# Jisu-Linnea-Han/ClimateMachine.jl

Hardware: AMD Instinct MI355X
Metric: DG RHS DOF-updates/sec (higher is better)
Workload: dtype f64; 1 GPU; Held-Suarez dry GCM (BASELINE configs[2]), stacked cubed sphere 6x30x30x8 elements, N=4, LSRK54 explicit, hyperdiffusion (DryBiharmonic, horizontal), Rusanov, fp64; elements=43200, nodes_per_element=125, states=5, parallelism=element partition (Hilbert, whole columns), 1 rank(s), RCCL p2p halo

## Files before the change

climatemachine.jl_amd/csrc/cmdg.hip:

```cpp
#include <dlfcn.h>

#include <algorithm>
#include <new>
#include <tuple>

#include "lapfused_tables.h"
#include "rccl.h"
#include "stepping.h"

namespace cmdg {

namespace {
typedef int (*roctx_push_t)(const char *);
typedef int (*roctx_pop_t)();
roctx_push_t g_roctx_push = nullptr;
roctx_pop_t g_roctx_pop = nullptr;
int g_roctx_state = 0;
void roctx_resolve()
{
    g_roctx_state = -1;
    const char *names[] = {"librocprofiler-sdk-roctx.so.1", "librocprofiler-sdk-roctx.so", "libroctx64.so.4",
                           "libroctx64.so", nullptr};
    const char *want = getenv("CMDG_ROCTX");
    void *lib = nullptr;
// ... 95 lines not shown
        m.first->eng->err.clear();
    }
    dev.emplace(named[0].first->eng);
}

int GroupCall::finish(int rc)
{
    if (rc == CMDG_OK) return rc;
    std::string msg = cmdg_status_string(rc);
    for (auto &m : members)
        if (!m.first->eng->err.empty()) {
            msg = m.second + m.first->eng->err;
            break;
        }
    for (auto &m : members) m.first->err = msg;
    return rc;
}

EngineBase::~EngineBase()
{
    delete worker;
    worker = nullptr;
    if (s_comp) hipStreamSynchronize(s_comp);
    if (s_comm) hipStreamSynchronize(s_comm);
    prof_collect();
    if (graph_exec) hipGraphExecDestroy(graph_exec);
    if (nccl_comm && rccl::CommDestroy) rccl::CommDestroy(nccl_comm);
}

static __global__ void k_face_digest(const double *__restrict__ vgeo, int nvgeo,
                                     const double *__restrict__ sgeo,
                                     const int64_t *__restrict__ vmapM,
                                     const int64_t *__restrict__ vmapP,
                                     const int64_t *__restrict__ elemtobndy, int NQ, int NQV,
                                     int64_t nreal, int32_t *__restrict__ faceP,
                                     double *__restrict__ faceG, double *__restrict__ faceW,
                                     int32_t *__restrict__ facePr, int *__restrict__ bad)
{
    const int Np = NQ * NQ * NQV, Nfph = NQ * NQV, Nfpv = NQ * NQ;
    const int Nfp = Nfph > Nfpv ? Nfph : Nfpv, NFT = 4 * Nfph + 2 * Nfpv;
    const int64_t I = (int64_t)blockIdx.x * blockDim.x + threadIdx.x;
    if (I >= nreal * NFT) return;
    const int64_t e = I / NFT;
    const int t = (int)(I % NFT);
    int f, n;
    if (t < 4 * Nfph) {
        f = t / Nfph;
        n = t % Nfph;
    } else {
        f = 4 + (t - 4 * Nfph) / Nfpv;
        n = (t - 4 * Nfph) % Nfpv;
    }
    const int64_t o = n + (int64_t)Nfp * (f + 6 * e);
    const int a = n % NQ, b = n / NQ;
    int vid;
    switch (f) {
    case 0: vid = NQ * (a + NQ * b); break;
    case 1: vid = (NQ - 1) + NQ * (a + NQ * b); break;
    case 2: vid = a + NQ * NQ * b; break;
    case 3: vid = a + NQ * ((NQ - 1) + NQ * b); break;
    case 4: vid = n; break;
    default: vid = n + NQ * NQ * (NQV - 1); break;
    }
    int flags = 0;
    const int64_t idM = vmapM[o] - 1;
    if (idM != e * Np + vid) flags |= 1;
    int64_t idP = vmapP[o] - 1;
    if (elemtobndy[f + 6 * e] != 0) idP = e * Np + vid;
    if (idP < 0 || idP > 2147483647LL) flags |= 4;
    faceP[I] = (int32_t)idP;
    const int64_t eP = idP >= 0 ? idP / Np : 0;
    facePr[I] = (int32_t)(eP * Np + ring_slot_of(NQ, NQV, (int)(idP - eP * Np)));
    const double *sg = sgeo + 5 * o;
#pragma unroll
    for (int c = 0; c < 4; ++c) faceG[((int64_t)4 * e + c) * NFT + t] = sg[c];
    const double mi = vgeo[vid + (int64_t)Np * (VMI + (int64_t)nvgeo * e)];
    if (!(sg[SVMI] == mi)) flags |= 2;
    faceW[I] = mi * sg[SSM];
    if (flags) atomicOr(bad, flags);
}

static __global__ void k_lapfused_fill(const double *__restrict__ vgeo, int nvgeo, const int32_t *__restrict__ faceP,
                                       const double *__restrict__ faceG, const double *__restrict__ faceW,
                                       const int32_t *__restrict__ lapI, int Np, int NFT, int NL, int64_t nreal,
                                       double *__restrict__ lapT)
{
    const int64_t I = (int64_t)blockIdx.x * blockDim.x + threadIdx.x;
    if (I >= nreal * NL) return;
    const int64_t e = I / NL;
    const int t = (int)(I % NL);
    const int64_t idP = faceP[NFT * e + t], N = idP / Np;
    const int vidP = (int)(idP - N * Np), tP = lapI[(2 * e + 0) * NL + t];
    const double *vg = vgeo + (int64_t)Np * nvgeo * N + vidP;
    const int rows[6] = {XI1X1, XI1X2, XI1X3, XI2X1, XI2X2, XI2X3};
    double *dst = lapT + 10 * e * NL + t;
#pragma unroll
    for (int c = 0; c < 6; ++c) dst[(int64_t)c * NL] = vg[(int64_t)rows[c] * Np];
#pragma unroll
    for (int c = 0; c < 3; ++c) dst[(int64_t)(6 + c) * NL] = faceG[((int64_t)4 * N + c) * NFT + tP];
    dst[(int64_t)9 * NL] = faceW[NFT * N + tP];
}

int EngineBase::init_lapfused()
{
    if (!garg_capable() || ngl <= 0 || nhyp != 3 * ngl || diffusion_direction != DIR_HORIZONTAL || nghost != 0 ||
        communicate() || fv || esdg || nreal < 1)
        return CMDG_OK;
    const int NFT = 4 * NQ * NQV + 2 * NQ * NQ, NL = 4 * NQ * NQV;
    std::vector<int32_t> h_faceP((size_t)(nreal * NFT));
    std::vector<int64_t> h_bndy((size_t)(6 * nreal));
    HIPCHK(hipMemcpy(h_faceP.data(), d_faceP, sizeof(int32_t) * h_faceP.size(), hipMemcpyDeviceToHost));
    HIPCHK(hipMemcpy(h_bndy.data(), g.elemtobndy, sizeof(int64_t) * h_bndy.size(), hipMemcpyDeviceToHost));
    LapFusedTables tab;
    lapfused_build(NQ, NQV, nreal, h_faceP.data(), h_bndy.data(), tab);
    if (!tab.eligible) return CMDG_OK;
    std::vector<int32_t> h_lapI((size_t)(2 * NL * nreal));
    for (int64_t e = 0; e < nreal; ++e)
        for (int t = 0; t < NL; ++t) {
            h_lapI[(size_t)((2 * e + 0) * NL + t)] = tab.tP[(size_t)(NL * e + t)];
            h_lapI[(size_t)((2 * e + 1) * NL + t)] = tab.tE[(size_t)(NL * e + t)];
        }
    HIPCHK(d_lapI.alloc(h_lapI.size()));
    HIPCHK(d_lapT.alloc((size_t)(10 * NL * nreal)));
    HIPCHK(hipMemcpy(d_lapI, h_lapI.data(), sizeof(int32_t) * h_lapI.size(), hipMemcpyHostToDevice));
    hipLaunchKernelGGL(k_lapfused_fill, dim3((unsigned)((nreal * NL + 255) / 256)), dim3(256), 0, s_comp, g.vgeo,
                       g.nvgeo, d_faceP.get(), d_faceG.get(), d_faceW.get(), d_lapI.get(), Np, NFT, NL, nreal,
                       d_lapT.get());
    if (hipGetLastError() != hipSuccess || hipStreamSynchronize(s_comp) != hipSuccess)
        return fail(CMDG_ERR_HIP, "cmdg_create: the tables of the fused Laplacian pass failed");
    lapfused_ok = true;
    return CMDG_OK;
}

int EngineBase::init(const cmdg_desc *d)
{
    Np = NQ * NQ * NQV;
    Nfp = NQ * (NQ > NQV ? NQ : NQV);
    if (d->N[0] != d->N[1] || d->N[0] != NQ - 1 || d->N[2] != NQV - 1)
        return fail(CMDG_ERR_INVALID, "cmdg_create: polynomial orders do not match the engine");
    if (NQV != NQ && !d->Dv)
        return fail(CMDG_ERR_INVALID, "cmdg_create: Dv is required when the vertical order differs");
    nreal = d->nreal;
    nghost = d->nghost;
    nelem = nreal + nghost;
    nf_first = d->nf_first;
    direction = d->direction;
    diffusion_direction = d->diffusion_direction;
    stacked = d->stacked;
    if (!d->vgeo || !d->sgeo || !d->vmapM || !d->vmapP || !d->elemtobndy || !d->D ||
        !d->state_auxiliary)
        return fail(CMDG_ERR_INVALID, "cmdg_create: a required grid/state pointer is NULL");
    if (d->nvgeo < 11) return fail(CMDG_ERR_INVALID, "cmdg_create: vgeo needs >= 11 columns");
    if (d->ninterior + d->nexterior != nreal)
        return fail(CMDG_ERR_INVALID, "cmdg_create: interior + exterior != nreal");
    if ((d->ninterior > 0 && !d->interiorelems) || (d->nexterior > 0 && !d->exteriorelems))
        return fail(CMDG_ERR_INVALID, "cmdg_create: element list pointer is NULL");
    if (direction < 0 || direction > 2 || diffusion_direction < 0 || diffusion_direction > 2)
        return fail(CMDG_ERR_INVALID, "cmdg_create: bad direction");
    g.vgeo = d->vgeo;
    g.sgeo = d->sgeo;
    g.vmapM = d->vmapM;
    g.vmapP = d->vmapP;
    g.elemtobndy = d->elemtobndy;
    g.nvgeo = d->nvgeo;
    d_interior = d_interior_user = d->interiorelems;
    ninterior = d->ninterior;
    d_exterior = d_exterior_user = d->exteriorelems;
    nexterior = d->nexterior;
    d_activedofs = d->activedofs;
    d_vmapsend = d->vmapsend;
    nvmapsend = d->nvmapsend;
    d_vmaprecv = d->vmaprecv;
    nvmaprecv = d->nvmaprecv;
    if (d->nnabr > 0) {
        if (!d->nabrtorank || !d->nabrtovmapsend || !d->nabrtovmaprecv || !d->vmapsend ||
            !d->vmaprecv)
            return fail(CMDG_ERR_INVALID, "cmdg_create: halo tables missing");
        nabrtorank.assign(d->nabrtorank, d->nabrtorank + d->nnabr);
        nabrsend.assign(d->nabrtovmapsend, d->nabrtovmapsend + 2 * d->nnabr);
        nabrrecv.assign(d->nabrtovmaprecv, d->nabrtovmaprecv + 2 * d->nnabr);
    }
    HIPCHK(hipGetDevice(&dev));
    HIPCHK(s_comp.create(hipStreamNonBlocking));
    {
        int lo = 0, hi = 0;
        const char *pv = getenv("CMDG_HALO_PRIORITY");
        if (communicate() && pv && *pv == '1' && hipDeviceGetStreamPriorityRange(&lo, &hi) == hipSuccess && hi < lo)
            HIPCHK(s_comm.create(hipStreamNonBlocking, hi));
        else
            HIPCHK(s_comm.create(hipStreamNonBlocking));
    }
    for (int i = 0; i < 2; ++i) {
        HIPCHK(ev_int[i].create(hipEventDisableTiming));
        HIPCHK(ev_ext[i].create(hipEventDisableTiming));
    }
    HIPCHK(gev_fork.create(hipEventDisableTiming));
    if (const char *v = getenv("CMDG_STEP_GRAPH")) step_graph = *v && *v != '0';
    HIPCHK(ev_comp.create(hipEventDisableTiming));
    HIPCHK(d_D.alloc(NQ * NQ));
    HIPCHK(hipMemcpy(d_D, d->D, sizeof(double) * NQ * NQ, hipMemcpyHostToDevice));
    g.D = d_D;
    g.Dv = d_D;
    if (NQV != NQ) {
        HIPCHK(d_Dv.alloc(NQV * NQV));
        HIPCHK(hipMemcpy(d_Dv, d->Dv, sizeof(double) * NQV * NQV, hipMemcpyHostToDevice));
        g.Dv = d_Dv;
    }
    {
        const int NFT = 4 * NQ * NQV + 2 * NQ * NQ;
// ... 764 lines not shown
```

climatemachine.jl_amd/csrc/kernels.h:

```cpp
#pragma once
#include "cmdg_common.h"
#include "law_defaults.h"

#ifndef CMDG_TEND_MINW
#define CMDG_TEND_MINW 1
#endif
#ifndef CMDG_TEND_EPB_LARGE
#define CMDG_TEND_EPB_LARGE 2
#endif
#ifndef CMDG_TEND_EPB_SMALL
#define CMDG_TEND_EPB_SMALL 1
#endif
#ifndef CMDG_GRAD_MINW
#define CMDG_GRAD_MINW 4
#endif
#ifndef CMDG_GRAD_BOUND_LARGE
#define CMDG_GRAD_BOUND_LARGE 1024
#endif
#ifndef CMDG_LAP_MINW
#define CMDG_LAP_MINW 1
#endif
#ifndef CMDG_LAPFUSED_MINW
#define CMDG_LAPFUSED_MINW 4
#endif
#ifndef CMDG_LAPFUSED_STAGE
#define CMDG_LAPFUSED_STAGE(idx, dep) asm volatile("" : "+v"(idx) : "v"(dep))
#endif

namespace cmdg {

template <class P>
struct PassArgs {
    typename P::Params prm;
    GridDev g;
    const int64_t *elems;
    int64_t nelems;
    const double *Q;
    const double *aux;
    double *aux_rw;
    const double *derived;
    double *gf;
    double *hypgrad;
    double *hypdiv;
    double *tendency;
    double *Qout;
    double *garg;
    double *lapr;
    int hypdiv_out;
    double t, alpha, beta;
    const double *tptr;
    double rkb_dt, rka_next;
    int direction;
    int model_dir;
    int nf_first;
    HaloDev h;
};

struct FacePt {
    double n[3], sM, vMI;
    double w;
    int64_t eP;
    int vidM, vidP, bctag;
};

template <int NQ, int NQV = NQ>
__host__ __device__ __forceinline__ constexpr int face_vid(int f, int n)
{
    const int a = n % NQ, b = n / NQ;
    switch (f) {
    case 0: return NQ * (a + NQ * b);
    case 1: return (NQ - 1) + NQ * (a + NQ * b);
    case 2: return a + NQ * NQ * b;
    case 3: return a + NQ * ((NQ - 1) + NQ * b);
    case 4: return n;
    default: return n + NQ * NQ * (NQV - 1);
    }
}

template <int NQ, int NQV = NQ>
__device__ __forceinline__ void face_index(const GridDev &g, int64_t e, int t, int f, int32_t &idP,
                                           int &bctag)
{
    idP = g.faceP[(int64_t)KDims<NQ, NQV>::NFT * e + t];
    bctag = (int)g.elemtobndy[f + 6 * e];
}
template <int NQ, int NQV = NQ, bool LIFTW = false>
__device__ __forceinline__ void face_geometry(const GridDev &g, int64_t e, int t, int f, int n,
                                              int32_t idP, int bctag, FacePt &fp)
{
    constexpr int Np = KDims<NQ, NQV>::Np, NFT = KDims<NQ, NQV>::NFT;
    const double *sg = g.faceG + (int64_t)4 * NFT * e + t;
    fp.n[0] = sg[0];
    fp.n[1] = sg[NFT];
    fp.n[2] = sg[2 * NFT];
    fp.vidM = face_vid<NQ, NQV>(f, n);
    if constexpr (LIFTW) {
        fp.w = g.faceW[(int64_t)NFT * e + t];
    } else {
        fp.sM = sg[3 * NFT];
        fp.vMI = g.vgeo[fp.vidM + (int64_t)Np * (VMI + (int64_t)g.nvgeo * e)];
    }
    fp.bctag = bctag;
    fp.eP = idP / Np;
    fp.vidP = idP - (int)fp.eP * Np;
}
template <int NQ, int NQV = NQ, bool LIFTW = false>
__device__ __forceinline__ void face_setup(const GridDev &g, int64_t e, int t, int f, int n,
                                           FacePt &fp)
{
// ... 793 lines not shown
                sC[(1 * NG + s) * Np + tid] = contravariant(M, x21, x22, x23, G1, G2, G3);
            }
            if (vt) sC[(2 * NG + s) * Np + tid] = contravariant(M, x31, x32, x33, G1, G2, G3);
            const int sidx = surf_index<NQ, NQV>(tid);
            if (sidx >= 0) {
                sM[(3 * s + 0) * NSURF + sidx] = G1;
                sM[(3 * s + 1) * NSURF + sidx] = G2;
                sM[(3 * s + 2) * NSURF + sidx] = G3;
            }
        }
    }
    __syncthreads();
    if (tid < Np) {
        const int i = tid % NQ, j = (tid / NQ) % NQ, k = tid / (NQ * NQ);
#pragma unroll
        for (int s = 0; s < NGL; ++s) {
            double dh = 0.0, dv = 0.0;
            if (hz) dh = div_volume_h<NQ>(MI, sD, sC + (0 * NG + s) * Np, sC + (1 * NG + s) * Np, i, j, k);
            if (vt) {
#pragma unroll
                for (int kk = 0; kk < NQV; ++kk)
                    dv -= MI * sDv[kk + NQV * k] * sC[(2 * NG + s) * Np + i + NQ * (j + NQ * kk)];
            }
            sA[s * Np + tid] = hz ? (vt ? dh + dv : dh) : dv;
        }
    }
    __syncthreads();
    Vec<NGL> corr;
    int vidM = 0, fpair = -1;
    if (tid < KD::NFT) {
        int f, n;
        KD::face_task(tid, f, n);
        const bool on = f < 4 ? hz : vt;
        if (on) {
            FacePt fp;
            face_setup<NQ, NQV, true>(a.g, e, tid, f, n, fp);
            Vec<NHG> gM, gP;
            const int sidx = surf_index<NQ, NQV>(fp.vidM);
#pragma unroll
            for (int q = 0; q < NHG; ++q) gM[q] = sM[q * NSURF + sidx];
            load_plus_hg<NHG, Np, NHG>(gP, a.hypgrad, a.h.recvHG, ghost_slot<Np>(a.h, fp.eP, fp.vidP),
                                    fp.vidP, fp.eP);
            if (fp.bctag != 0) {
                Vec<NAUX> auxM, auxP;
                load_state<NAUX, Np>(auxM, a.aux, fp.vidM, e);
                load_state<NAUX, Np>(auxP, a.aux, fp.vidP, fp.eP);
                P::boundary_state_divergence(a.prm, fp.bctag, gP, auxP, fp.n, gM, auxM, a_t);
            }
            const double nh0 = fp.n[0] / 2, nh1 = fp.n[1] / 2, nh2 = fp.n[2] / 2;
#pragma unroll
            for (int s = 0; s < NGL; ++s) {
                const double ldiv = central_divergence_flux(&gP[3 * s], &gM[3 * s], nh0, nh1, nh2);
                corr[s] = fp.w * ldiv;
            }
            vidM = fp.vidM;
            fpair = f / 2;
        }
    }
#pragma unroll
    for (int p = 0; p < 3; ++p) {
        if (fpair == p) {
#pragma unroll
            for (int s = 0; s < NGL; ++s) sA[s * Np + vidM] += corr[s];
        }
        __syncthreads();
    }
    if constexpr (RING) store_ring_major<NG, NQ, NQV>(a.lapr, e, tid, (int)blockDim.x, sA);
    if (tid < Np) {
        if (!RING || a.hypdiv_out) {
#pragma unroll
            for (int s = 0; s < NGL; ++s)
                a.hypdiv[tid + (int64_t)Np * (s + (int64_t)NHYP * e)] = sA[s * Np + tid];
        }
    }
    if constexpr (NGL > 0)
        send_nodes<NGL, NGL>(a.h, 0, e, tid, (int)blockDim.x, [&](int s, int n) { return sA[s * Np + n]; });
}

template <class P, int NQ, int NQV = NQ>
__global__ void __launch_bounds__((KDims<NQ, NQV>::NT), CMDG_LAPFUSED_MINW) k_lapfused(const PassArgs<P> a)
{
    using KD = KDims<NQ, NQV>;
    constexpr int Np = KD::Np, NGL = P::NGL, NHG = 3 * NGL, NHYP = P::NHYP, NG = NGL > 0 ? NGL : 1,
                  NFT = KD::NFT, NL = 4 * KD::Nfph, NT = KD::NT;
    static_assert(NT >= NL && NGL > 0, "one lane per lateral face task");
    __shared__ double sD[NQ * NQ];
    __shared__ double sG[NG * Np];
    __shared__ double sA[3 * NG * Np];
    __shared__ double sC[2 * NG * Np];
    __shared__ double sL[NG * Np];
    const int tid = threadIdx.x;
    const int64_t e = a.elems[xcd_remap(blockIdx.x, gridDim.x)] - 1;
    const int ft = tid - (NT - NL);
    if (tid < NQ * NQ) sD[tid] = a.g.D[tid];
    if (tid < Np) {
        const double *rec = a.garg + garg_at<NGL, Np>(tid, e);
        Vec<NGL> r;
#pragma unroll
        for (int s = 0; s < NGL; ++s) r[s] = rec[s];
#pragma unroll
        for (int s = 0; s < NGL; ++s) sG[s * Np + tid] = r[s];
    }
    FacePt fp;
    int tP = 0, tE = -1, iP = 0, jP = 0, kP = 0;
    int32_t idE = 0;
    const double *gN = a.garg;
    if (ft >= 0) {
        int f, n;
        KD::face_task(ft, f, n);
        face_setup<NQ, NQV, true>(a.g, e, ft, f, n, fp);
        tP = a.g.facePr[((int64_t)2 * e + 0) * NL + ft];
        tE = a.g.facePr[((int64_t)2 * e + 1) * NL + ft];
        gN = a.garg + garg_at<NGL, Np>(0, fp.eP);
        iP = fp.vidP % NQ, jP = (fp.vidP / NQ) % NQ, kP = fp.vidP / (NQ * NQ);
        if (tE >= 0) idE = a.g.faceP[(int64_t)NFT * fp.eP + tE];
    }
    double M = 0, MI = 0, x11 = 0, x12 = 0, x13 = 0, x21 = 0, x22 = 0, x23 = 0;
    if (tid < Np) {
        const double *vg = a.g.vgeo + (int64_t)Np * a.g.nvgeo * e + tid;
        M = vg[VM * Np];
        MI = vg[VMI * Np];
        x11 = vg[XI1X1 * Np], x12 = vg[XI1X2 * Np], x13 = vg[XI1X3 * Np];
        x21 = vg[XI2X1 * Np], x22 = vg[XI2X2 * Np], x23 = vg[XI2X3 * Np];
    }
    __syncthreads();
    if (tid < Np) {
        const int i = tid % NQ, j = (tid / NQ) % NQ, k = tid / (NQ * NQ);
        Vec<NHG> gh;
        gh.negzero();
#pragma unroll
        for (int s = 0; s < NGL; ++s)
            grad_volume_h<NQ>(
                sD, i, j, [&](int n) { return sG[s * Np + n + NQ * (j + NQ * k)]; },
                [&](int n) { return sG[s * Np + i + NQ * (n + NQ * k)]; }, x11, x12, x13, x21, x22, x23, &gh[3 * s]);
#pragma unroll
        for (int q = 0; q < NHG; ++q) sA[q * Np + tid] = gh[q];
    }
    Vec<NHG> corr, gP;
    int fpair = -1;
    if (ft >= 0) {
        fpair = ft / (2 * KD::Nfph);
        const double *lapT = a.derived + (int64_t)10 * NL * e + ft;
        Vec<NGL> GY, G1, G2;
        double r1[NQ][NG];
#pragma unroll
        for (int s = 0; s < NGL; ++s) GY[s] = gN[NGL * fp.vidP + s];
#pragma unroll
        for (int n = 0; n < NQ; ++n)
#pragma unroll
            for (int s = 0; s < NGL; ++s) r1[n][s] = gN[NGL * (n + NQ * (jP + NQ * kP)) + s];
#pragma unroll
        for (int s = 0; s < NGL; ++s) G1[s] = line_derivative<NQ>(sD, iP, [&](int n) { return r1[n][s]; });
#pragma unroll
        for (int s = 0; s < NGL; ++s) CMDG_LAPFUSED_STAGE(kP, G1[s]);
        double r2[NQ][NG];
#pragma unroll
        for (int n = 0; n < NQ; ++n)
#pragma unroll
            for (int s = 0; s < NGL; ++s) r2[n][s] = gN[NGL * (iP + NQ * (n + NQ * kP)) + s];
        double T[6];
#pragma unroll
        for (int c = 0; c < 6; ++c) T[c] = lapT[c * NL];
#pragma unroll
        for (int s = 0; s < NGL; ++s) G2[s] = line_derivative<NQ>(sD, jP, [&](int n) { return r2[n][s]; });
        gP.negzero();
#pragma unroll
        for (int s = 0; s < NGL; ++s) metric_gradient(T[0], T[1], T[2], T[3], T[4], T[5], G1[s], G2[s], &gP[3 * s]);
#pragma unroll
        for (int q = 0; q < NHG; ++q) CMDG_LAPFUSED_STAGE(idE, gP[q]);
        double nS[3], wS, nE[3] = {0, 0, 0}, wE = 0;
#pragma unroll
        for (int d = 0; d < 3; ++d) nS[d] = lapT[(6 + d) * NL];
        wS = lapT[9 * NL];
        Vec<NGL> GE;
        int pairE = 2;
        if (tE >= 0) {
            const double *sg = a.g.faceG + (int64_t)4 * NFT * fp.eP + tE;
            nE[0] = sg[0], nE[1] = sg[NFT], nE[2] = sg[2 * NFT];
            wE = a.g.faceW[(int64_t)NFT * fp.eP + tE];
            const double *rec = a.garg + (int64_t)NGL * idE;
#pragma unroll
            for (int s = 0; s < NGL; ++s) GE[s] = rec[s];
            int fE, nn;
            KD::face_task(tE, fE, nn);
            pairE = fE / 2;
        }
        int fS, nn;
        KD::face_task(tP, fS, nn);
        const bool edge_first = pairE < fS / 2;
        Vec<NGL> GM;
#pragma unroll
        for (int s = 0; s < NGL; ++s) GM[s] = sG[s * Np + fp.vidM];
#pragma unroll
        for (int s = 0; s < NGL; ++s)
#pragma unroll
            for (int d = 0; d < 3; ++d) {
                const double lS = gradient_lift(wS, central_gradient_flux(nS[d], GM[s], GY[s]), nS[d] * GY[s]);
                if (tE >= 0) {
                    const double lE = gradient_lift(wE, central_gradient_flux(nE[d], GE[s], GY[s]), nE[d] * GY[s]);
                    gP[3 * s + d] += edge_first ? lE : lS;
                    gP[3 * s + d] += edge_first ? lS : lE;
                } else {
                    gP[3 * s + d] += lS;
                }
            }
#pragma unroll
        for (int s = 0; s < NGL; ++s)
#pragma unroll
            for (int d = 0; d < 3; ++d)
                corr[3 * s + d] =
                    gradient_lift(fp.w, central_gradient_flux(fp.n[d], GY[s], GM[s]), fp.n[d] * GM[s]);
    }
    __syncthreads();
#pragma unroll
    for (int p = 0; p < 2; ++p) {
        if (fpair == p) {
#pragma unroll
            for (int q = 0; q < NHG; ++q) sA[q * Np + fp.vidM] += corr[q];
        }
        __syncthreads();
    }
    if (tid < Np) {
#pragma unroll
        for (int s = 0; s < NGL; ++s) {
            const double G1 = sA[(3 * s + 0) * Np + tid], G2 = sA[(3 * s + 1) * Np + tid],
                         G3 = sA[(3 * s + 2) * Np + tid];
            sC[(0 * NG + s) * Np + tid] = contravariant(M, x11, x12, x13, G1, G2, G3);
            sC[(1 * NG + s) * Np + tid] = contravariant(M, x21, x22, x23, G1, G2, G3);
        }
    }
    __syncthreads();
    if (tid < Np) {
        const int i = tid % NQ, j = (tid / NQ) % NQ, k = tid / (NQ * NQ);
#pragma unroll
        for (int s = 0; s < NGL; ++s)
            sL[s * Np + tid] = div_volume_h<NQ>(MI, sD, sC + (0 * NG + s) * Np, sC + (1 * NG + s) * Np, i, j, k);
    }
    Vec<NGL> corrL;
    if (ft >= 0) {
        Vec<NHG> gM;
#pragma unroll
        for (int q = 0; q < NHG; ++q) gM[q] = sA[q * Np + fp.vidM];
        const double nh0 = fp.n[0] / 2, nh1 = fp.n[1] / 2, nh2 = fp.n[2] / 2;
#pragma unroll
        for (int s = 0; s < NGL; ++s) {
            const double ldiv = central_divergence_flux(&gP[3 * s], &gM[3 * s], nh0, nh1, nh2);
            corrL[s] = fp.w * ldiv;
        }
    }
    __syncthreads();
#pragma unroll
    for (int p = 0; p < 2; ++p) {
        if (fpair == p) {
#pragma unroll
            for (int s = 0; s < NGL; ++s) sL[s * Np + fp.vidM] += corrL[s];
        }
        __syncthreads();
    }
    store_ring_major<NG, NQ, NQV>(a.lapr, e, tid, (int)blockDim.x, sL);
    if (tid < Np && a.hypdiv_out) {
#pragma unroll
        for (int s = 0; s < NGL; ++s) a.hypdiv[tid + (int64_t)Np * (s + (int64_t)NHYP * e)] = sL[s * Np + tid];
    }
}

template <class P, int NQ, int NQV = NQ, bool RING = false>
__global__ void __launch_bounds__((KDims<NQ, NQV>::NT), CMDG_LAP_MINW) k_gradlap(const PassArgs<P> a)
{
    using KD = KDims<NQ, NQV>;
    const double a_t = a.tptr ? *a.tptr : a.t;
    constexpr int Np = KD::Np, NS = P::NS, NAUX = P::NAUX, NGL = P::NGL,
                  NHG = 3 * NGL, NHYP = P::NHYP, NG = NGL > 0 ? NGL : 1,
                  NH = NHYP > 0 ? NHYP : 1;
    __shared__ double sD[NQ * NQ + (NQV == NQ ? 0 : NQV * NQV)];
    const double *const sDv = sD + (NQV == NQ ? 0 : NQ * NQ);
    __shared__ double sL[NG * Np];
    __shared__ double sA[NH * Np];
    const int tid = threadIdx.x;
    const int64_t e = a.elems[xcd_remap(blockIdx.x, gridDim.x)] - 1;
    if (tid < NQ * NQ) sD[tid] = a.g.D[tid];
    if constexpr (NQV != NQ) {
        if (tid < NQV * NQV) sD[NQ * NQ + tid] = a.g.Dv[tid];
    }
    const bool hz = a.direction != DIR_VERTICAL, vt = a.direction != DIR_HORIZONTAL;
    if (tid < Np) {
        Vec<NGL> l;
        if constexpr (RING) {
            const double *rec = a.lapr + garg_at<NG, Np>(ring_slot<NQ, NQV>(tid), e);
#pragma unroll
            for (int s = 0; s < NGL; ++s) l[s] = rec[s];
        } else {
#pragma unroll
            for (int s = 0; s < NGL; ++s) l[s] = a.hypdiv[tid + (int64_t)Np * (s + (int64_t)NHYP * e)];
        }
#pragma unroll
        for (int s = 0; s < NGL; ++s) sL[s * Np + tid] = l[s];
    }
    __syncthreads();
    if (tid < Np) {
        const int i = tid % NQ, j = (tid / NQ) % NQ, k = tid / (NQ * NQ);
        const double *vg = a.g.vgeo + (int64_t)Np * a.g.nvgeo * e + tid;
        Vec<NS> lQ;
        Vec<NAUX> laux;
        load_state<NS, Np>(lQ, a.Q, tid, e);
        load_state<NAUX, Np>(laux, a.aux, tid, e);
        Vec<NHG> lh, lv;
        lh.negzero();
        lv.negzero();
        if (hz) {
            const double x11 = vg[XI1X1 * Np], x12 = vg[XI1X2 * Np], x13 = vg[XI1X3 * Np];
            const double x21 = vg[XI2X1 * Np], x22 = vg[XI2X2 * Np], x23 = vg[XI2X3 * Np];
#pragma unroll
            for (int s = 0; s < NGL; ++s) {
                double l1 = 0.0, l2 = 0.0;
#pragma unroll
                for (int n = 0; n < NQ; ++n) {
                    l1 += sD[i + NQ * n] * sL[s * Np + n + NQ * (j + NQ * k)];
                    l2 += sD[j + NQ * n] * sL[s * Np + i + NQ * (n + NQ * k)];
                }
                lh[3 * s + 0] = x11 * l1;
                lh[3 * s + 1] = x12 * l1;
                lh[3 * s + 2] = x13 * l1;
// ... 322 lines not shown
```

climatemachine.jl_amd/csrc/lapfused_tables.h:

```cpp
#pragma once
#include <stdint.h>

#include <string>
#include <vector>

namespace cmdg {

struct LapFusedTables {
    int NQ = 0, NQV = 0;
    int64_t nreal = 0;
    bool eligible = false;
    std::string why;
    std::vector<int32_t> tP, tE;
};

inline int lapfused_face_vid(int NQ, int NQV, int t)
{
    const int Nfph = NQ * NQV, f = t / Nfph, n = t % Nfph, a = n % NQ, b = n / NQ;
    switch (f) {
    case 0: return NQ * (a + NQ * b);
    case 1: return (NQ - 1) + NQ * (a + NQ * b);
    case 2: return a + NQ * NQ * b;
    default: return a + NQ * ((NQ - 1) + NQ * b);
    }
}

inline void lapfused_tasks_of(int NQ, int NQV, int vid, int out[2])
{
    const int Nfph = NQ * NQV, i = vid % NQ, j = (vid / NQ) % NQ, k = vid / (NQ * NQ);
    out[0] = i == 0 ? j + NQ * k : (i == NQ - 1 ? Nfph + j + NQ * k : -1);
    out[1] = j == 0 ? 2 * Nfph + i + NQ * k : (j == NQ - 1 ? 3 * Nfph + i + NQ * k : -1);
}

inline void lapfused_build(int NQ, int NQV, int64_t nreal, const int32_t *faceP, const int64_t *elemtobndy,
                           LapFusedTables &out)
{
    out = LapFusedTables();
    out.NQ = NQ;
    out.NQV = NQV;
    out.nreal = nreal;
    auto no = [&](const std::string &m) {
        out.eligible = false;
        out.why = m;
        out.tP.clear();
        out.tE.clear();
    };
    if (NQ < 2 || NQV < 1 || nreal < 1 || !faceP || !elemtobndy) return no("empty grid");
    const int Np = NQ * NQ * NQV, Nfph = NQ * NQV, NL = 4 * Nfph, NFT = NL + 2 * NQ * NQ;
    auto str = [](int64_t v) { return std::to_string(v); };
    for (int64_t e = 0; e < nreal; ++e)
        for (int f = 0; f < 4; ++f)
            if (elemtobndy[f + 6 * e] != 0)
                return no("lateral face " + str(f + 1) + " of element " + str(e + 1) + " is a boundary face");
    out.tP.assign((size_t)(NL * nreal), -1);
    out.tE.assign((size_t)(NL * nreal), -1);
    for (int64_t e = 0; e < nreal; ++e)
        for (int t = 0; t < NL; ++t) {
            const int64_t idP = faceP[NFT * e + t];
            const int64_t me = e * Np + lapfused_face_vid(NQ, NQV, t);
            if (idP < 0 || idP >= nreal * Np)
                return no("face task " + str(t) + " of element " + str(e + 1) + " has no real element on its plus side");
            const int64_t N = idP / Np;
            int cand[2];
            lapfused_tasks_of(NQ, NQV, (int)(idP - N * Np), cand);
            int found = -1, other = -1, matches = 0;
            for (int c = 0; c < 2; ++c) {
                if (cand[c] < 0) continue;
                if (faceP[NFT * N + cand[c]] == me) {
                    if (matches++ == 0) found = cand[c];
                } else {
                    other = cand[c];
                }
            }
            if (matches != 1)
                return no("face task " + str(t) + " of element " + str(e + 1) + (matches == 0 ? " is not seen" : " is seen twice") +
                          " from its neighbour " + str(N + 1));
            out.tP[(size_t)(NL * e + t)] = found;
            out.tE[(size_t)(NL * e + t)] = other;
        }
    out.eligible = true;
}

}
```

Measured before the change: 22.05 billion DOF-updates/s.

## Share neighbour face-row values via LDS and precompute edge geometry in fused Laplacian

The fused Laplacian kernel now loads only the neighbour's normal line per face lane and shares the along-face values through a new LDS buffer, so the tangential derivative comes from LDS instead of a second strided global gather. Edge-neighbour normals, weights and record indices are precomputed into the per-element table, replacing the dependent faceP/faceG lookups at run time. Loads are hoisted ahead of the first barrier, and the manual asm staging macros are replaced with simple register pins. The host builder adds checks that each face row maps to a single neighbour row, which could make some grids ineligible for this path, and the extra LDS buffer may change occupancy.

Result: faster. 22.54 billion DOF-updates/s (median of 6 runs) (+2.2%).

```diff
diff --git a/climatemachine.jl_amd/csrc/cmdg.hip b/climatemachine.jl_amd/csrc/cmdg.hip
--- a/climatemachine.jl_amd/csrc/cmdg.hip
+++ b/climatemachine.jl_amd/csrc/cmdg.hip
@@ -201,23 +201,30 @@
 
 static __global__ void k_lapfused_fill(const double *__restrict__ vgeo, int nvgeo, const int32_t *__restrict__ faceP,
                                        const double *__restrict__ faceG, const double *__restrict__ faceW,
-                                       const int32_t *__restrict__ lapI, int Np, int NFT, int NL, int64_t nreal,
-                                       double *__restrict__ lapT)
-{
+                                       const int32_t *__restrict__ lapI, const int32_t *__restrict__ tE_of, int NQ,
+                                       int NQV, int64_t nreal, double *__restrict__ lapT)
+{
+    const int Np = NQ * NQ * NQV, Nfph = NQ * NQV, NL = 4 * Nfph, NFT = NL + 2 * NQ * NQ, NE = 8 * NQV;
     const int64_t I = (int64_t)blockIdx.x * blockDim.x + threadIdx.x;
     if (I >= nreal * NL) return;
     const int64_t e = I / NL;
     const int t = (int)(I % NL);
     const int64_t idP = faceP[NFT * e + t], N = idP / Np;
-    const int vidP = (int)(idP - N * Np), tP = lapI[(2 * e + 0) * NL + t];
+    const int vidP = (int)(idP - N * Np), tP = lapI[(2 * e + 0) * NL + t], tE = tE_of[I];
     const double *vg = vgeo + (int64_t)Np * nvgeo * N + vidP;
     const int rows[6] = {XI1X1, XI1X2, XI1X3, XI2X1, XI2X2, XI2X3};
-    double *dst = lapT + 10 * e * NL + t;
+    double *dst = lapT + (int64_t)(10 * NL + 4 * NE) * e + t;
 #pragma unroll
     for (int c = 0; c < 6; ++c) dst[(int64_t)c * NL] = vg[(int64_t)rows[c] * Np];
 #pragma unroll
     for (int c = 0; c < 3; ++c) dst[(int64_t)(6 + c) * NL] = faceG[((int64_t)4 * N + c) * NFT + tP];
     dst[(int64_t)9 * NL] = faceW[NFT * N + tP];
+    if (tE < 0) return;
+    const bool last = lapfused_index_in_face(NQ, tP / Nfph, vidP) == NQ - 1;
+    double *edge = lapT + (int64_t)(10 * NL + 4 * NE) * e + 10 * NL + lapfused_edge_slot(NQV, t / Nfph, (t % Nfph) / NQ, last);
+#pragma unroll
+    for (int c = 0; c < 3; ++c) edge[c * NE] = faceG[((int64_t)4 * N + c) * NFT + tE];
+    edge[3 * NE] = faceW[NFT * N + tE];
 }
 
 int EngineBase::init_lapfused()
@@ -237,13 +244,16 @@
     for (int64_t e = 0; e < nreal; ++e)
         for (int t = 0; t < NL; ++t) {
             h_lapI[(size_t)((2 * e + 0) * NL + t)] = tab.tP[(size_t)(NL * e + t)];
-            h_lapI[(size_t)((2 * e + 1) * NL + t)] = tab.tE[(size_t)(NL * e + t)];
-        }
+            h_lapI[(size_t)((2 * e + 1) * NL + t)] = tab.idE[(size_t)(NL * e + t)];
+        }
+    DevBuf<int32_t> d_tE;
     HIPCHK(d_lapI.alloc(h_lapI.size()));
-    HIPCHK(d_lapT.alloc((size_t)(10 * NL * nreal)));
+    HIPCHK(d_tE.alloc(tab.tE.size()));
+    HIPCHK(d_lapT.alloc((size_t)((10 * NL + 4 * 8 * NQV) * nreal)));
     HIPCHK(hipMemcpy(d_lapI, h_lapI.data(), sizeof(int32_t) * h_lapI.size(), hipMemcpyHostToDevice));
+    HIPCHK(hipMemcpy(d_tE, tab.tE.data(), sizeof(int32_t) * tab.tE.size(), hipMemcpyHostToDevice));
     hipLaunchKernelGGL(k_lapfused_fill, dim3((unsigned)((nreal * NL + 255) / 256)), dim3(256), 0, s_comp, g.vgeo,
-                       g.nvgeo, d_faceP.get(), d_faceG.get(), d_faceW.get(), d_lapI.get(), Np, NFT, NL, nreal,
+                       g.nvgeo, d_faceP.get(), d_faceG.get(), d_faceW.get(), d_lapI.get(), d_tE.get(), NQ, NQV, nreal,
                        d_lapT.get());
     if (hipGetLastError() != hipSuccess || hipStreamSynchronize(s_comp) != hipSuccess)
         return fail(CMDG_ERR_HIP, "cmdg_create: the tables of the fused Laplacian pass failed");
diff --git a/climatemachine.jl_amd/csrc/kernels.h b/climatemachine.jl_amd/csrc/kernels.h
--- a/climatemachine.jl_amd/csrc/kernels.h
+++ b/climatemachine.jl_amd/csrc/kernels.h
@@ -22,9 +22,6 @@
 #endif
 #ifndef CMDG_LAPFUSED_MINW
 #define CMDG_LAPFUSED_MINW 4
-#endif
-#ifndef CMDG_LAPFUSED_STAGE
-#define CMDG_LAPFUSED_STAGE(idx, dep) asm volatile("" : "+v"(idx) : "v"(dep))
 #endif
 
 namespace cmdg {
@@ -984,46 +981,66 @@
 {
     using KD = KDims<NQ, NQV>;
     constexpr int Np = KD::Np, NGL = P::NGL, NHG = 3 * NGL, NHYP = P::NHYP, NG = NGL > 0 ? NGL : 1,
-                  NFT = KD::NFT, NL = 4 * KD::Nfph, NT = KD::NT;
+                  NL = 4 * KD::Nfph, NT = KD::NT, NE = 8 * NQV, LT = 10 * NL + 4 * NE;
     static_assert(NT >= NL && NGL > 0, "one lane per lateral face task");
     __shared__ double sD[NQ * NQ];
     __shared__ double sG[NG * Np];
     __shared__ double sA[3 * NG * Np];
     __shared__ double sC[2 * NG * Np];
     __shared__ double sL[NG * Np];
+    __shared__ double sX[NG * NL];
+    static_assert(sizeof(double) * (NQ * NQ + 7 * NG * Np + NG * NL) <= 32768,
+                  "LDS of k_lapfused: five work-groups per CU");
     const int tid = threadIdx.x;
     const int64_t e = a.elems[xcd_remap(blockIdx.x, gridDim.x)] - 1;
     const int ft = tid - (NT - NL);
     if (tid < NQ * NQ) sD[tid] = a.g.D[tid];
+    Vec<NGL> r;
+    double M = 0, MI = 0, x11 = 0, x12 = 0, x13 = 0, x21 = 0, x22 = 0, x23 = 0;
+#pragma unroll
+    for (int s = 0; s < NGL; ++s) r[s] = 0;
     if (tid < Np) {
         const double *rec = a.garg + garg_at<NGL, Np>(tid, e);
-        Vec<NGL> r;
 #pragma unroll
         for (int s = 0; s < NGL; ++s) r[s] = rec[s];
-#pragma unroll
-        for (int s = 0; s < NGL; ++s) sG[s * Np + tid] = r[s];
-    }
-    FacePt fp;
-    int tP = 0, tE = -1, iP = 0, jP = 0, kP = 0;
-    int32_t idE = 0;
-    const double *gN = a.garg;
+        const double *vg = a.g.vgeo + (int64_t)Np * a.g.nvgeo * e + tid;
+        M = vg[VM * Np];
+        MI = vg[VMI * Np];
+        x11 = vg[XI1X1 * Np], x12 = vg[XI1X2 * Np], x13 = vg[XI1X3 * Np];
+        x21 = vg[XI2X1 * Np], x22 = vg[XI2X2 * Np], x23 = vg[XI2X3 * Np];
+    }
+    FacePt fp = {};
+    int32_t idE = -1;
+    int tP = 0;
     if (ft >= 0) {
         int f, n;
         KD::face_task(ft, f, n);
         face_setup<NQ, NQV, true>(a.g, e, ft, f, n, fp);
         tP = a.g.facePr[((int64_t)2 * e + 0) * NL + ft];
-        tE = a.g.facePr[((int64_t)2 * e + 1) * NL + ft];
-        gN = a.garg + garg_at<NGL, Np>(0, fp.eP);
-        iP = fp.vidP % NQ, jP = (fp.vidP / NQ) % NQ, kP = fp.vidP / (NQ * NQ);
-        if (tE >= 0) idE = a.g.faceP[(int64_t)NFT * fp.eP + tE];
-    }
-    double M = 0, MI = 0, x11 = 0, x12 = 0, x13 = 0, x21 = 0, x22 = 0, x23 = 0;
+        idE = a.g.facePr[((int64_t)2 * e + 1) * NL + ft];
+    }
+    asm volatile("" ::"v"(M), "v"(MI), "v"(x11), "v"(x12), "v"(x13), "v"(x21), "v"(x22), "v"(x23), "v"(r[0]),
+                 "v"(r[NGL - 1]), "v"(fp.vidP), "v"(fp.w), "v"(fp.n[0]), "v"(fp.n[1]), "v"(fp.n[2]), "v"(tP), "v"(idE));
     if (tid < Np) {
-        const double *vg = a.g.vgeo + (int64_t)Np * a.g.nvgeo * e + tid;
-        M = vg[VM * Np];
-        MI = vg[VMI * Np];
-        x11 = vg[XI1X1 * Np], x12 = vg[XI1X2 * Np], x13 = vg[XI1X3 * Np];
-        x21 = vg[XI2X1 * Np], x22 = vg[XI2X2 * Np], x23 = vg[XI2X3 * Np];
+#pragma unroll
+        for (int s = 0; s < NGL; ++s) sG[s * Np + tid] = r[s];
+    }
+    int idx = 0, xrow = 0;
+    bool x1 = true, far = false;
+    double rn[NQ][NG] = {};
+    if (ft >= 0) {
+        int fS, nn;
+        KD::face_task(tP, fS, nn);
+        x1 = fS < 2, far = fS & 1;
+        const int iP = fp.vidP % NQ, jP = (fp.vidP / NQ) % NQ, kP = fp.vidP / (NQ * NQ);
+        idx = x1 ? jP : iP;
+        xrow = ft - ft % NQ;
+        const double *line = a.garg + garg_at<NGL, Np>(x1 ? NQ * (jP + NQ * kP) : iP + NQ * NQ * kP, fp.eP);
+        const int step = x1 ? NGL : NGL * NQ;
+#pragma unroll
+        for (int m = 0; m < NQ; ++m)
+#pragma unroll
+            for (int s = 0; s < NGL; ++s) rn[m][s] = line[m * step + s];
     }
     __syncthreads();
     if (tid < Np) {
@@ -1038,67 +1055,92 @@
 #pragma unroll
         for (int q = 0; q < NHG; ++q) sA[q * Np + tid] = gh[q];
     }
-    Vec<NHG> corr, gP;
+    Vec<NHG> corr;
+    Vec<NGL> Gn;
     int fpair = -1;
     if (ft >= 0) {
         fpair = ft / (2 * KD::Nfph);
-        const double *lapT = a.derived + (int64_t)10 * NL * e + ft;
-        Vec<NGL> GY, G1, G2;
-        double r1[NQ][NG];
-#pragma unroll
-        for (int s = 0; s < NGL; ++s) GY[s] = gN[NGL * fp.vidP + s];
-#pragma unroll
-        for (int n = 0; n < NQ; ++n)
-#pragma unroll
-            for (int s = 0; s < NGL; ++s) r1[n][s] = gN[NGL * (n + NQ * (jP + NQ * kP)) + s];
-#pragma unroll
-        for (int s = 0; s < NGL; ++s) G1[s] = line_derivative<NQ>(sD, iP, [&](int n) { return r1[n][s]; });
-#pragma unroll
-        for (int s = 0; s < NGL; ++s) CMDG_LAPFUSED_STAGE(kP, G1[s]);
-        double r2[NQ][NG];
-#pragma unroll
-        for (int n = 0; n < NQ; ++n)
-#pragma unroll
-            for (int s = 0; s < NGL; ++s) r2[n][s] = gN[NGL * (iP + NQ * (n + NQ * kP)) + s];
-        double T[6];
-#pragma unroll
-        for (int c = 0; c < 6; ++c) T[c] = lapT[c * NL];
-#pragma unroll
-        for (int s = 0; s < NGL; ++s) G2[s] = line_derivative<NQ>(sD, jP, [&](int n) { return r2[n][s]; });
+        Vec<NGL> GY, GM;
+#pragma unroll
+        for (int s = 0; s < NGL; ++s) GY[s] = far ? rn[NQ - 1][s] : rn[0][s];
+#pragma unroll
+        for (int s = 0; s < NGL; ++s) sX[s * NL + xrow + idx] = GY[s];
+#pragma unroll
+        for (int s = 0; s < NGL; ++s) GM[s] = sG[s * Np + fp.vidM];
+#pragma unroll
+        for (int s = 0; s < NGL; ++s)
+            Gn[s] = line_derivative<NQ>(sD, far ? NQ - 1 : 0, [&](int m) { return rn[m][s]; });
+#pragma unroll
+        for (int s = 0; s < NGL; ++s)
+#pragma unroll
+            for (int d = 0; d < 3; ++d)
+                corr[3 * s + d] =
+                    gradient_lift(fp.w, central_gradient_flux(fp.n[d], GY[s], GM[s]), fp.n[d] * GM[s]);
+    }
+    __syncthreads();
+#pragma unroll
+    for (int m = 0; m < NQ; ++m) asm volatile("" ::"v"(rn[m][0]), "v"(rn[m][NGL - 1]));
+#pragma unroll
+    for (int p = 0; p < 2; ++p) {
+        if (fpair == p) {
+#pragma unroll
+            for (int q = 0; q < NHG; ++q) sA[q * Np + fp.vidM] += corr[q];
+        }
+        __syncthreads();
+    }
+    double T[10], nE[3] = {0, 0, 0}, wE = 0;
+    Vec<NGL> GE;
+    if (ft >= 0) {
+        const double *lapT = a.derived + (int64_t)LT * e;
+#pragma unroll
+        for (int c = 0; c < 10; ++c) T[c] = lapT[c * NL + ft];
+        if (idE >= 0) {
+            const double *edge = lapT + 10 * NL + 2 * (ft / NQ) + (idx == NQ - 1 ? 1 : 0);
+            nE[0] = edge[0], nE[1] = edge[NE], nE[2] = edge[2 * NE];
+            wE = edge[3 * NE];
+            const double *rec = a.garg + (int64_t)NGL * idE;
+#pragma unroll
+            for (int s = 0; s < NGL; ++s) GE[s] = rec[s];
+        }
+    }
+    if (tid < Np) {
+#pragma unroll
+        for (int s = 0; s < NGL; ++s) {
+            const double G1 = sA[(3 * s + 0) * Np + tid], G2 = sA[(3 * s + 1) * Np + tid],
+                         G3 = sA[(3 * s + 2) * Np + tid];
+            sC[(0 * NG + s) * Np + tid] = contravariant(M, x11, x12, x13, G1, G2, G3);
+            sC[(1 * NG + s) * Np + tid] = contravariant(M, x21, x22, x23, G1, G2, G3);
+        }
+    }
+    __syncthreads();
+    if (tid < Np) {
+        const int i = tid % NQ, j = (tid / NQ) % NQ, k = tid / (NQ * NQ);
+#pragma unroll
+        for (int s = 0; s < NGL; ++s)
+            sL[s * Np + tid] = div_volume_h<NQ>(MI, sD, sC + (0 * NG + s) * Np, sC + (1 * NG + s) * Np, i, j, k);
+    }
+    Vec<NGL> corrL;
+    if (ft >= 0) {
+        Vec<NGL> GY, GM, Gf;
+#pragma unroll
+        for (int s = 0; s < NGL; ++s) GY[s] = sX[s * NL + xrow + idx];
+#pragma unroll
+        for (int s = 0; s < NGL; ++s) GM[s] = sG[s * Np + fp.vidM];
+#pragma unroll
+        for (int s = 0; s < NGL; ++s)
+            Gf[s] = line_derivative<NQ>(sD, idx, [&](int m) { return sX[s * NL + xrow + m]; });
+        Vec<NHG> gP;
         gP.negzero();
 #pragma unroll
-        for (int s = 0; s < NGL; ++s) metric_gradient(T[0], T[1], T[2], T[3], T[4], T[5], G1[s], G2[s], &gP[3 * s]);
-#pragma unroll
-        for (int q = 0; q < NHG; ++q) CMDG_LAPFUSED_STAGE(idE, gP[q]);
-        double nS[3], wS, nE[3] = {0, 0, 0}, wE = 0;
-#pragma unroll
-        for (int d = 0; d < 3; ++d) nS[d] = lapT[(6 + d) * NL];
-        wS = lapT[9 * NL];
-        Vec<NGL> GE;
-        int pairE = 2;
-        if (tE >= 0) {
-            const double *sg = a.g.faceG + (int64_t)4 * NFT * fp.eP + tE;
-            nE[0] = sg[0], nE[1] = sg[NFT], nE[2] = sg[2 * NFT];
-            wE = a.g.faceW[(int64_t)NFT * fp.eP + tE];
-            const double *rec = a.garg + (int64_t)NGL * idE;
-#pragma unroll
-            for (int s = 0; s < NGL; ++s) GE[s] = rec[s];
-            int fE, nn;
-            KD::face_task(tE, fE, nn);
-            pairE = fE / 2;
-        }
-        int fS, nn;
-        KD::face_task(tP, fS, nn);
-        const bool edge_first = pairE < fS / 2;
-        Vec<NGL> GM;
-#pragma unroll
-        for (int s = 0; s < NGL; ++s) GM[s] = sG[s * Np + fp.vidM];
-#pragma unroll
         for (int s = 0; s < NGL; ++s)
+            metric_gradient(T[0], T[1], T[2], T[3], T[4], T[5], x1 ? Gn[s] : Gf[s], x1 ? Gf[s] : Gn[s], &gP[3 * s]);
+        const bool edge_first = !x1;
+#pragma unroll
+        for (int s = 0; s < NGL; ++s)
 #pragma unroll
             for (int d = 0; d < 3; ++d) {
-                const double lS = gradient_lift(wS, central_gradient_flux(nS[d], GM[s], GY[s]), nS[d] * GY[s]);
-                if (tE >= 0) {
+                const double lS = gradient_lift(T[9], central_gradient_flux(T[6 + d], GM[s], GY[s]), T[6 + d] * GY[s]);
+                if (idE >= 0) {
                     const double lE = gradient_lift(wE, central_gradient_flux(nE[d], GE[s], GY[s]), nE[d] * GY[s]);
                     gP[3 * s + d] += edge_first ? lE : lS;
                     gP[3 * s + d] += edge_first ? lS : lE;
@@ -1106,40 +1148,6 @@
                     gP[3 * s + d] += lS;
                 }
             }
-#pragma unroll
-        for (int s = 0; s < NGL; ++s)
-#pragma unroll
-            for (int d = 0; d < 3; ++d)
-                corr[3 * s + d] =
-                    gradient_lift(fp.w, central_gradient_flux(fp.n[d], GY[s], GM[s]), fp.n[d] * GM[s]);
-    }
-    __syncthreads();
-#pragma unroll
-    for (int p = 0; p < 2; ++p) {
-        if (fpair == p) {
-#pragma unroll
-            for (int q = 0; q < NHG; ++q) sA[q * Np + fp.vidM] += corr[q];
-        }
-        __syncthreads();
-    }
-    if (tid < Np) {
-#pragma unroll
-        for (int s = 0; s < NGL; ++s) {
-            const double G1 = sA[(3 * s + 0) * Np + tid], G2 = sA[(3 * s + 1) * Np + tid],
-                         G3 = sA[(3 * s + 2) * Np + tid];
-            sC[(0 * NG + s) * Np + tid] = contravariant(M, x11, x12, x13, G1, G2, G3);
-            sC[(1 * NG + s) * Np + tid] = contravariant(M, x21, x22, x23, G1, G2, G3);
-        }
-    }
-    __syncthreads();
-    if (tid < Np) {
-        const int i = tid % NQ, j = (tid / NQ) % NQ, k = tid / (NQ * NQ);
-#pragma unroll
-        for (int s = 0; s < NGL; ++s)
-            sL[s * Np + tid] = div_volume_h<NQ>(MI, sD, sC + (0 * NG + s) * Np, sC + (1 * NG + s) * Np, i, j, k);
-    }
-    Vec<NGL> corrL;
-    if (ft >= 0) {
         Vec<NHG> gM;
 #pragma unroll
         for (int q = 0; q < NHG; ++q) gM[q] = sA[q * Np + fp.vidM];
diff --git a/climatemachine.jl_amd/csrc/lapfused_tables.h b/climatemachine.jl_amd/csrc/lapfused_tables.h
--- a/climatemachine.jl_amd/csrc/lapfused_tables.h
+++ b/climatemachine.jl_amd/csrc/lapfused_tables.h
@@ -3,6 +3,12 @@
 
 #include <string>
 #include <vector>
+
+#ifdef __HIPCC__
+#define CMDG_LAPFUSED_HD __host__ __device__
+#else
+#define CMDG_LAPFUSED_HD
+#endif
 
 namespace cmdg {
 
@@ -12,7 +18,17 @@
     bool eligible = false;
     std::string why;
     std::vector<int32_t> tP, tE;
+    std::vector<int32_t> idE;
 };
+
+CMDG_LAPFUSED_HD inline int lapfused_edge_slot(int NQV, int f, int b, bool last)
+{
+    return 2 * (f * NQV + b) + (last ? 1 : 0);
+}
+CMDG_LAPFUSED_HD inline int lapfused_index_in_face(int NQ, int f, int vid)
+{
+    return f < 2 ? (vid / NQ) % NQ : vid % NQ;
+}
 
 inline int lapfused_face_vid(int NQ, int NQV, int t)
 {
@@ -44,6 +60,7 @@
         out.why = m;
         out.tP.clear();
         out.tE.clear();
+        out.idE.clear();
     };
     if (NQ < 2 || NQV < 1 || nreal < 1 || !faceP || !elemtobndy) return no("empty grid");
     const int Np = NQ * NQ * NQV, Nfph = NQ * NQV, NL = 4 * Nfph, NFT = NL + 2 * NQ * NQ;
@@ -54,6 +71,7 @@
                 return no("lateral face " + str(f + 1) + " of element " + str(e + 1) + " is a boundary face");
     out.tP.assign((size_t)(NL * nreal), -1);
     out.tE.assign((size_t)(NL * nreal), -1);
+    out.idE.assign((size_t)(NL * nreal), -1);
     for (int64_t e = 0; e < nreal; ++e)
         for (int t = 0; t < NL; ++t) {
             const int64_t idP = faceP[NFT * e + t];
@@ -77,6 +95,25 @@
                           " from its neighbour " + str(N + 1));
             out.tP[(size_t)(NL * e + t)] = found;
             out.tE[(size_t)(NL * e + t)] = other;
+            if (other >= 0) out.idE[(size_t)(NL * e + t)] = faceP[NFT * N + other];
+        }
+    for (int64_t e = 0; e < nreal; ++e)
+        for (int r = 0; r < 4 * NQV; ++r) {
+            const int f = r / NQV, b = r % NQV, t0 = f * Nfph + NQ * b;
+            const std::string row = "the row of face " + str(f + 1) + ", level " + str(b + 1) + " of element " + str(e + 1);
+            const int64_t N0 = faceP[NFT * e + t0] / Np;
+            const int k0 = (int)(faceP[NFT * e + t0] - N0 * Np) / (NQ * NQ), f0 = out.tP[(size_t)(NL * e + t0)] / Nfph;
+            unsigned seen = 0;
+            for (int a = 0; a < NQ; ++a) {
+                const int64_t idP = faceP[NFT * e + t0 + a], N = idP / Np;
+                const int vidP = (int)(idP - N * Np);
+                if (N != N0) return no(row + " straddles two neighbours");
+                if (vidP / (NQ * NQ) != k0) return no(row + " straddles two levels of its neighbour");
+                const unsigned bit = 1u << lapfused_index_in_face(NQ, f0, vidP);
+                if (seen & bit) return no(row + " repeats an index along its neighbour's face");
+                seen |= bit;
+                if (out.tP[(size_t)(NL * e + t0 + a)] / Nfph != f0) return no(row + " straddles two faces of its neighbour");
+            }
         }
     out.eligible = true;
 }
```
